# SobeyMIL/MVOC

Hardware: AMD Instinct MI355X
Metric: UNet3D denoising steps/sec, 16x512^2 frames, inversion+compose (higher is better)
Workload: dtype f16

## Files before the change

mvoc_amd/csrc/attention.hip:

```cpp
#include <stdlib.h>

#include "common.h"

namespace {

typedef __fp16 fp16x4_t __attribute__((__vector_size__(4 * sizeof(__fp16))));
template <int D> struct FlashPitch { static constexpr int K = 2 * D + 16, V = D == 64 ? 192 : 320; };

struct AttnArgs {
  const half_t *q, *k, *v;
  half_t* out;
  long q_bs, q_ts, k_bs, k_ts, v_bs, v_ts, o_bs, o_ts;
  int nbatch, heads, tq, tk, kv_bdiv, causal;
  float scale_log2;
  long v2_off, o2_off;
  int qblocks;
};

__device__ __forceinline__ int vt_slot_group(int key) {
  return ((((key >> 5) * 2 + ((key >> 4) & 1)) * 2) + ((key >> 2) & 1));
}
__device__ __forceinline__ int vt_slot_elem(int key) { return ((key >> 3) & 1) * 4 + (key & 3); }

constexpr float FLASH_THR = 8.0f;
// ... 298 lines not shown
      for (int e = 0; e < 16; ++e) ot[v][dt][e] = 0.f;
  float mrun = -INFINITY, lrun = 0.f;
  f32x16 sa[2], sb[2];
  f32x16 zero16;
#pragma unroll
  for (int e = 0; e < 16; ++e) zero16[e] = 0.f;

  int kfo[4];
#pragma unroll
  for (int s = 0; s < 4; ++s) kfo[s] = r * 128 + (((2 * s + h) ^ ((r >> 1) & 7)) * 16);
  const int vq = (lane & 15) >> 2;
  int vfo[2];
#pragma unroll
  for (int dt = 0; dt < 2; ++dt) vfo[dt] = 8192 + (4 * h + vq) * 128 + (((32 * ((lane >> 4) & 1) + 8 * (lane & 3))) | ((dt ^ ((vq >> 1) & 1)) << 6));

  f3_wait_vm<(NS - 2) * PCS>();
  F3_BAR();
#pragma unroll
  for (int t = 0; t < 2; ++t) {
    sa[t] = zero16;
#pragma unroll
    for (int s = 0; s < 4; ++s) {
      const half8_t kf = *reinterpret_cast<const half8_t*>(smem + kfo[s] + 4096 * t);
      sa[t] = __builtin_amdgcn_mfma_f32_32x32x16_f16(kf, qf[s], sa[t], 0, 0, 0);
    }
  }
  int o_v = 0, o_k = TILE, o_w = (NS - 1) * TILE;

  auto body = [&](f32x16(&cur)[2], f32x16(&nxt)[2], const int t) {
    F3_STAMP(4);
    f3_wait_vm<(NS - 3) * PCS>();
    F3_BAR();
    F3_STAMP(0);
    issue(t + NS - 1, o_w);
    F3_FENCE();
    F3_STAMP(1);
    const char* Kn = smem + o_k;
    const char* Vc = smem + o_v;
    if (__builtin_amdgcn_readfirstlane((t == nt - 1) && (p.tk & 63))) {
#pragma unroll
      for (int tt = 0; tt < 2; ++tt)
#pragma unroll
        for (int e = 0; e < 16; ++e)
          if (t * 64 + 32 * tt + 8 * (e >> 2) + 4 * h + (e & 3) >= p.tk) cur[tt][e] = -INFINITY;
    }
    F3_FENCE();
    half8_t kf[2][4];
#pragma unroll
    for (int s = 0; s < 2; ++s)
#pragma unroll
      for (int tt = 0; tt < 2; ++tt) kf[tt][s] = *reinterpret_cast<const half8_t*>(Kn + kfo[s] + 4096 * tt);
    half8_t pf[2];
    half8_t vf[3][NV][2];
    auto vread = [&](const int f) {
#pragma unroll
      for (int v = 0; v < NV; ++v)
#pragma unroll
        for (int dt = 0; dt < 2; ++dt) {
          const char* va = Vc + 8192 * v + vfo[dt] + (32 * (f >> 1) + 16 * (f & 1)) * 128;
          const fp16x4_t lo = __builtin_amdgcn_ds_read_tr16_b64_v4f16((__attribute__((address_space(3))) fp16x4_t*)va);
          const fp16x4_t hi = __builtin_amdgcn_ds_read_tr16_b64_v4f16((__attribute__((address_space(3))) fp16x4_t*)(va + 8 * 128));
#pragma unroll
          for (int e = 0; e < 4; ++e) {
            vf[f % 3][v][dt][e] = (half_t)lo[e];
            vf[f % 3][v][dt][4 + e] = (half_t)hi[e];
          }
        }
    };
    vread(0);
    F3_FENCE();
    auto smma = [&](const int i) {
      const int tt = i & 1, s_ = i >> 1;
      nxt[tt] = __builtin_amdgcn_mfma_f32_32x32x16_f16(kf[tt][s_], qf[s_], s_ == 0 ? zero16 : nxt[tt], 0, 0, 0);
    };
    auto pvmma = [&](const int f, const int dt) {
#pragma unroll
      for (int v = 0; v < NV; ++v) ot[v][dt] = __builtin_amdgcn_mfma_f32_32x32x16_f16(vf[f % 3][v][dt], pf[f & 1], ot[v][dt], 0, 0, 0);
    };
    float mx = fmaxf(cur[0][0], cur[0][1]);
#pragma unroll
    for (int tt = 0; tt < 2; ++tt)
#pragma unroll
      for (int e = tt ? 0 : 2; e < 16; e += 2) mx = __builtin_fmaxf(__builtin_fmaxf(mx, cur[tt][e]), cur[tt][e + 1]);
    smma(0); smma(1); smma(2);
    if constexpr (NV == 2) smma(3);
    mx = flash_xhalf_max(mx);
    if constexpr (NV == 1) { F3_GRP(6, 0); F3_GRP(6, 0); F3_GRP(6, 0); }
    else { F3_GRP(4, 0); F3_GRP(5, 0); F3_GRP(4, 0); F3_GRP(5, 0); }
    F3_STAMP(2);
    if (__any((mx - mrun) * p.scale_log2 > FLASH_THR)) {
      const float mnew = fmaxf(mrun, mx);
      const float alpha = __builtin_amdgcn_exp2f((mrun - mnew) * p.scale_log2);
      mrun = mnew;
      lrun *= alpha;
#pragma unroll
      for (int v = 0; v < NV; ++v)
#pragma unroll
        for (int dt = 0; dt < 2; ++dt)
#pragma unroll
          for (int e = 0; e < 16; ++e) ot[v][dt][e] *= alpha;
    }
    F3_FENCE();
    const f32x2 sc2 = {p.scale_log2, p.scale_log2}, mc2 = {-mrun * p.scale_log2, -mrun * p.scale_log2};
#pragma unroll
    for (int s = 2; s < 4; ++s)
#pragma unroll
      for (int tt = 0; tt < 2; ++tt) kf[tt][s] = *reinterpret_cast<const half8_t*>(Kn + kfo[s] + 4096 * tt);
#pragma unroll
    for (int f = 0; f < 4; ++f) {
      const int tt = f >> 1, s_ = f & 1;
      if (f < 3) vread(f + 1);
      half8_t& pn = pf[f & 1];
      float x[8];
#pragma unroll
      for (int j = 0; j < 8; j += 2) {
        const f32x2 a = __builtin_elementwise_fma(f32x2{cur[tt][8 * s_ + j], cur[tt][8 * s_ + j + 1]}, sc2, mc2);
        x[j] = __builtin_amdgcn_exp2f(a[0]);
        x[j + 1] = __builtin_amdgcn_exp2f(a[1]);
      }
#pragma unroll
      for (int j = 0; j < 8; ++j) pn[j] = (half_t)x[j];
#pragma unroll
      for (int j = 0; j < 4; ++j) lrun = __builtin_amdgcn_fdot2(half2_t{pn[2 * j], pn[2 * j + 1]}, half2_t{(half_t)1.f, (half_t)1.f}, lrun, false);
      if (f == 0) {
        smma(NV == 1 ? 3 : 4); smma(NV == 1 ? 4 : 5);
        if constexpr (NV == 2) { smma(6); smma(7); } else smma(5);
      } else {
        pvmma(f - 1, 0); pvmma(f - 1, 1);
        if constexpr (NV == 1) { if (f < 3) smma(5 + f); }
      }
    }
    pvmma(3, 0);
    pvmma(3, 1);
    if constexpr (NV == 1) {
      F3_RD(8); F3_GRP(5, 3); F3_GRP(5, 2); F3_GRP(5, 3);
      F3_RD(4); F3_GRP(5, 2); F3_GRP(5, 3); F3_GRP(5, 2);
      F3_RD(4); F3_GRP(5, 3); F3_GRP(5, 2); F3_GRP(5, 3);
      F3_GRP(5, 2); F3_GRP(5, 3); F3_GRP(5, 2); F3_GRP(5, 2);
    } else {
      F3_RD(12); F3_GRP(3, 2); F3_GRP(3, 2); F3_GRP(3, 2); F3_GRP(3, 2);
      F3_RD(8); F3_GRP(3, 2); F3_GRP(3, 2); F3_GRP(3, 2); F3_GRP(3, 2);
      F3_RD(8); F3_GRP(3, 2); F3_GRP(3, 2); F3_GRP(3, 2); F3_GRP(3, 2);
      F3_GRP(3, 2); F3_GRP(3, 2); F3_GRP(3, 2); F3_GRP(3, 2);
      F3_GRP(3, 0); F3_GRP(3, 0); F3_GRP(3, 0); F3_GRP(3, 0);
    }
    F3_FENCE();
    F3_STAMP(3);
    const int o_ = o_v; o_v = o_k;
    o_k = o_k + TILE == NS * TILE ? 0 : o_k + TILE;
    o_w = o_;
  };
#pragma unroll 1
  for (int t = 0;; t += 2) {
    body(sa, sb, t);
    if (t + 1 >= nt) break;
    body(sb, sa, t + 1);
    if (t + 2 >= nt) break;
  }
  f3_wait_vm<0>();
#ifdef MVOC_F3_STAMPS
  if (blockIdx.x == 0 && tid == 0) {
    unsigned long long t1_, r1_;
    asm volatile("s_memtime %0\n\ts_memrealtime %1\n\ts_waitcnt lgkmcnt(0)" : "=s"(t1_), "=s"(r1_)::"memory");
    for (int i = 0; i < 5; ++i) f3_dbg[i] = f3_acc[i];
    f3_dbg[5] = t1_ - f3_t0;
    f3_dbg[7] = r1_ - f3_r0;
    f3_dbg[6] = (unsigned long long)nt;
  }
#endif

  const float ltot = lrun + __shfl_xor(lrun, 32);
  const float inv = 1.0f / ltot;
  if (q0 + r < p.tq) {
#pragma unroll
    for (int v = 0; v < NV; ++v) {
      half_t* op = p.out + v * p.o2_off + (long)b * p.o_bs + (long)(q0 + r) * p.o_ts + head * D;
#pragma unroll
      for (int dt = 0; dt < 2; ++dt)
#pragma unroll
        for (int q = 0; q < 4; ++q) {
          half4_t o;
#pragma unroll
          for (int e = 0; e < 4; ++e) o[e] = (half_t)(ot[v][dt][q * 4 + e] * inv);
          *reinterpret_cast<half4_t*>(op + 32 * dt + 8 * q + 4 * h) = o;
        }
    }
  }
}
#undef F3_BAR
#undef F3_FENCE
#undef F3_GRP
#undef F3_RD
#undef F3_STAMP

struct TAttnArgs {
  const half_t *q, *k, *v;
  half_t* out;
  long q_bs, q_ps, q_ts, k_bs, k_ps, k_ts, v_bs, v_ps, v_ts, o_bs, o_ps, o_ts;
  int nsample, hw, heads, frames;
  int logf, logp, pgroups;
  long ntask;
  float scale_log2;
};

constexpr int TVPITCH = 64;

__global__ __launch_bounds__(256) void tattn_kernel(const TAttnArgs p) {
  __shared__ __attribute__((aligned(16))) char smem[4 * 64 * TVPITCH];
  const int tid = threadIdx.x, lane = tid & 63, wave = tid >> 6;
  const int r = lane & 31, h = lane >> 5;
  char* Vs = smem + wave * 64 * TVPITCH;
  const int F = p.frames, logf = p.logf, P = 1 << p.logp;
  const long task = (long)blockIdx.x * 4 + wave;
  const bool active = task < p.ntask;
  const long tk = active ? task : p.ntask - 1;
  const int head = (int)(tk % p.heads);
  const long bp = tk / p.heads;
  const long smp = bp / p.pgroups, px0 = (bp % p.pgroups) << p.logp;
  const half8_t zero8 = {0, 0, 0, 0, 0, 0, 0, 0};
  auto row_px = [&](int row) { return (long)(P > 1 ? row >> logf : 0); };
  auto row_fr = [&](int row) { return P > 1 ? row & (F - 1) : row; };
  auto row_ok = [&](int row) { return (P > 1 || row < F) && px0 + row_px(row) < p.hw; };

  const half_t* qb = p.q + smp * p.q_bs + px0 * p.q_ps + head * 64;
  const half_t* kb = p.k + smp * p.k_bs + px0 * p.k_ps + head * 64;
  const half_t* vb = p.v + smp * p.v_bs + px0 * p.v_ps + head * 64;

#pragma unroll
  for (int i = 0; i < 4; ++i) {
    const int c = lane + 64 * i;
    const int key = c >> 3, dc = c & 7;
    half8_t vr = zero8;
    if (row_ok(key)) vr = *reinterpret_cast<const half8_t*>(vb + row_px(key) * p.v_ps + (long)row_fr(key) * p.v_ts + dc * 8);
    const int g = (((key >> 4) & 1) * 2) + ((key >> 2) & 1), j = vt_slot_elem(key);
#pragma unroll
    for (int e = 0; e < 8; ++e) {
      const int d = dc * 8 + e;
      *reinterpret_cast<half_t*>(Vs + d * TVPITCH + ((g ^ ((d >> 3) & 3)) * 16) + j * 2) = vr[e];
    }
  }
  f32x16 st;
#pragma unroll
  for (int e = 0; e < 16; ++e) st[e] = 0.f;
  const bool rok = row_ok(r);
  const long koff = row_px(r) * p.k_ps + (long)row_fr(r) * p.k_ts, qoff = row_px(r) * p.q_ps + (long)row_fr(r) * p.q_ts;
#pragma unroll
  for (int s = 0; s < 4; ++s) {
    half8_t kf = zero8, qf = zero8;
    if (rok) {
      kf = *reinterpret_cast<const half8_t*>(kb + koff + 16 * s + 8 * h);
      qf = *reinterpret_cast<const half8_t*>(qb + qoff + 16 * s + 8 * h);
    }
    st = __builtin_amdgcn_mfma_f32_32x32x16_f16(kf, qf, st, 0, 0, 0);
  }
  float mx = -INFINITY;
#pragma unroll
  for (int e = 0; e < 16; ++e) {
    const int key = 8 * (e >> 2) + 4 * h + (e & 3);
    const bool ok = P > 1 ? (key >> logf) == (r >> logf) : key < F;
    const float sv = ok ? st[e] * p.scale_log2 : -INFINITY;
    st[e] = sv;
    mx = fmaxf(mx, sv);
  }
  mx = fmaxf(mx, __shfl_xor(mx, 32));
  float ps = 0.f;
#pragma unroll
  for (int e = 0; e < 16; ++e) {
    const float pv = __builtin_amdgcn_exp2f(st[e] - mx);
    st[e] = pv;
    ps += pv;
  }
  ps += __shfl_xor(ps, 32);
  const float inv = 1.0f / ps;

  __syncthreads();
  f32x16 ot[2];
#pragma unroll
  for (int dt = 0; dt < 2; ++dt)
#pragma unroll
    for (int e = 0; e < 16; ++e) ot[dt][e] = 0.f;
#pragma unroll
  for (int s = 0; s < 2; ++s) {
    half8_t pf;
#pragma unroll
    for (int j = 0; j < 8; ++j) pf[j] = (half_t)st[8 * s + j];
    const int g = s * 2 + h;
#pragma unroll
    for (int dt = 0; dt < 2; ++dt) {
      const int d = 32 * dt + r;
      const half8_t vf = *reinterpret_cast<const half8_t*>(Vs + d * TVPITCH + ((g ^ ((d >> 3) & 3)) * 16));
      ot[dt] = __builtin_amdgcn_mfma_f32_32x32x16_f16(vf, pf, ot[dt], 0, 0, 0);
    }
  }
  if (active && rok) {
    half_t* op = p.out + smp * p.o_bs + (px0 + row_px(r)) * p.o_ps + (long)row_fr(r) * p.o_ts + head * 64;
#pragma unroll
    for (int dt = 0; dt < 2; ++dt)
#pragma unroll
      for (int q = 0; q < 4; ++q) {
        half4_t o;
#pragma unroll
        for (int e = 0; e < 4; ++e) o[e] = (half_t)(ot[dt][q * 4 + e] * inv);
        *reinterpret_cast<half4_t*>(op + 32 * dt + 8 * q + 4 * h) = o;
      }
  }
}

}

static const int g_f3_env = getenv("MVOC_FLASH3") ? atoi(getenv("MVOC_FLASH3")) : -1;

extern "C" int mvoc_flash_attn_f16(const mvoc_attn_desc* d, void* stream) {
  MVOC_REQUIRE(d && d->q && d->k && d->v && d->out, -1, "flash_attn: null operand");
  MVOC_REQUIRE(d->nbatch > 0 && d->heads > 0 && d->tq > 0 && d->tk > 0, -1, "flash_attn: empty problem");
  MVOC_REQUIRE(d->nbatch <= 65535 && d->heads <= 65535, -2, "flash_attn: grid too large");
  MVOC_REQUIRE(d->q_ts % 8 == 0 && d->k_ts % 8 == 0 && d->v_ts % 8 == 0 && d->o_ts % 4 == 0, -2,
               "flash_attn: row strides must keep 16-byte alignment");
  AttnArgs a;
  a.q = (const half_t*)d->q; a.k = (const half_t*)d->k; a.v = (const half_t*)d->v; a.out = (half_t*)d->out;
  a.q_bs = d->q_bs; a.q_ts = d->q_ts; a.k_bs = d->k_bs; a.k_ts = d->k_ts; a.v_bs = d->v_bs; a.v_ts = d->v_ts;
  a.o_bs = d->o_bs; a.o_ts = d->o_ts;
  a.nbatch = d->nbatch; a.heads = d->heads; a.tq = d->tq; a.tk = d->tk; a.kv_bdiv = d->kv_bdiv > 0 ? d->kv_bdiv : 1;
  const int hd = d->head_dim > 0 ? d->head_dim : 64;
  MVOC_REQUIRE(hd == 64 || hd == 96, -2, "flash_attn: head_dim (%d) must be 64 or 96", hd);
  MVOC_REQUIRE(!d->causal || d->tq == d->tk, -2, "flash_attn: the causal form is self-attention (tq == tk)");
  a.causal = d->causal;
  a.scale_log2 = (d->scale > 0.f ? d->scale : (hd == 64 ? 0.125f : 1.0f / sqrtf((float)hd))) * 1.4426950408889634f;
  hipStream_t s = (hipStream_t)stream;
  MvocProfScope prof(MVOC_FAM_FLASH, s, (d->v2 ? 2.0 : 1.0) * 4.0 * d->nbatch * d->heads * (double)d->tq * d->tk * hd);
  a.qblocks = (d->tq + 127) / 128;
  const long nblk = (long)a.qblocks * d->heads * d->nbatch;
  MVOC_REQUIRE(nblk < 0x7fffffffL, -2, "flash_attn: grid too large");
  dim3 grid((unsigned)nblk);
  a.v2_off = a.o2_off = 0;
  MVOC_REQUIRE(d->pipelined >= 0 && d->pipelined <= 2, -1, "flash_attn: pipelined must be 0 (by key count), 1 (never) or 2 (wherever it applies)");
  const int f3_mode = d->pipelined ? d->pipelined - 1 : g_f3_env;
  const bool pipelined = hd == 64 && !d->causal && (f3_mode >= 0 ? f3_mode != 0 : d->tk >= 2048);
  if (d->v2) {
    MVOC_REQUIRE(d->out2 && hd == 64, -2, "flash_attn: the paired form needs out2 and head_dim 64");
    a.v2_off = (const half_t*)d->v2 - a.v;
    a.o2_off = (half_t*)d->out2 - a.out;
    MVOC_REQUIRE(a.v2_off % 8 == 0 && a.o2_off % 4 == 0, -2, "flash_attn: v2 / out2 must keep 16-byte alignment");
    if (pipelined) hipLaunchKernelGGL((flash3_kernel<2>), grid, dim3(256), 0, s, a);
    else hipLaunchKernelGGL((flash_kernel<64, 2>), grid, dim3(256), 0, s, a);
  } else if (hd == 64) {
    if (pipelined) hipLaunchKernelGGL((flash3_kernel<1>), grid, dim3(256), 0, s, a);
    else hipLaunchKernelGGL((flash_kernel<64, 1>), grid, dim3(256), 0, s, a);
  } else {
    hipLaunchKernelGGL((flash_kernel<96, 1>), grid, dim3(256), 0, s, a);
  }
  return mvoc_check_launch("flash_kernel");
}

#ifdef MVOC_F3_STAMPS
extern "C" int mvoc_f3_stamps_read(unsigned long long* host8) {
  return hipMemcpyFromSymbol(host8, HIP_SYMBOL(f3_dbg), sizeof(unsigned long long) * 8) == hipSuccess ? 0 : -1;
}
#endif

extern "C" int mvoc_temporal_attn_f16(const mvoc_tattn_desc* d, void* stream) {
  MVOC_REQUIRE(d && d->q && d->k && d->v && d->out, -1, "temporal_attn: null operand");
  MVOC_REQUIRE(d->nsample > 0 && d->hw > 0 && d->heads > 0, -1, "temporal_attn: empty problem");
  MVOC_REQUIRE(d->frames >= 1 && d->frames <= 32, -2, "temporal_attn: frames (%d) must be in [1, 32]", d->frames);
  MVOC_REQUIRE(d->q_ts % 8 == 0 && d->k_ts % 8 == 0 && d->v_ts % 8 == 0 && d->o_ts % 4 == 0 && d->q_ps % 8 == 0 &&
                   d->k_ps % 8 == 0 && d->v_ps % 8 == 0 && d->o_ps % 4 == 0,
               -2, "temporal_attn: strides must keep 16-byte alignment");
  TAttnArgs a;
  a.q = (const half_t*)d->q; a.k = (const half_t*)d->k; a.v = (const half_t*)d->v; a.out = (half_t*)d->out;
  a.q_bs = d->q_bs; a.q_ps = d->q_ps; a.q_ts = d->q_ts; a.k_bs = d->k_bs; a.k_ps = d->k_ps; a.k_ts = d->k_ts;
  a.v_bs = d->v_bs; a.v_ps = d->v_ps; a.v_ts = d->v_ts; a.o_bs = d->o_bs; a.o_ps = d->o_ps; a.o_ts = d->o_ts;
  a.nsample = d->nsample; a.hw = d->hw; a.heads = d->heads; a.frames = d->frames;
  a.logf = d->frames == 8 ? 3 : d->frames == 16 ? 4 : 5;
  a.logp = d->frames == 8 ? 2 : d->frames == 16 ? 1 : 0;
  a.pgroups = (d->hw + (1 << a.logp) - 1) >> a.logp;
  a.ntask = (long)d->nsample * a.pgroups * d->heads;
  a.scale_log2 = 0.125f * 1.4426950408889634f;
  const long nblk = (a.ntask + 3) / 4;
  MVOC_REQUIRE(nblk < 0x7fffffffL, -2, "temporal_attn: grid too large");
  hipStream_t s = (hipStream_t)stream;
  MvocProfScope prof(MVOC_FAM_TATTN, s, 4.0 * (double)d->nsample * d->hw * d->heads * d->frames * 64 * 2);
  hipLaunchKernelGGL(tattn_kernel, dim3((unsigned)nblk), dim3(256), 0, s, a);
  return mvoc_check_launch("tattn_kernel");
}
```

mvoc_amd/csrc/stem.hip:

```cpp
#include "common.h"

namespace {

__global__ void timestep_embedding_kernel(const float* __restrict__ t, int nb, int dim, half_t* __restrict__ out) {
  const int i = blockIdx.x * blockDim.x + threadIdx.x;
  const int half = dim / 2;
  if (i >= nb * dim) return;
  const int b = i / dim, j = i % dim;
  const int k = j < half ? j : j - half;
  const float freq = expf(-logf(10000.0f) * (float)k / (float)half);
  const float ang = t[b] * freq;
  out[i] = (half_t)(j < half ? cosf(ang) : sinf(ang));
}

__global__ void act_kernel(const half_t* __restrict__ x, half_t* __restrict__ out, long n, int act) {
  const long i = (long)blockIdx.x * blockDim.x + threadIdx.x;
  if (i >= n) return;
  const float v = (float)x[i];
  out[i] = (half_t)(act == MVOC_ACT_SILU ? silu_f(v) : act == MVOC_ACT_GELU ? gelu_erf_f(v) : v);
}

__global__ void add_kernel(const half_t* __restrict__ a, const half_t* __restrict__ b, half_t* __restrict__ out, long n) {
  const long i = (long)blockIdx.x * blockDim.x + threadIdx.x;
  if (i >= n) return;
  out[i] = (half_t)((float)a[i] + (float)b[i]);
}

__global__ void conv3x3_small_kernel(const half_t* __restrict__ x, const half_t* __restrict__ w,
                                     const half_t* __restrict__ bias, half_t* __restrict__ out, int nimg, int h, int wd,
                                     int cin, int cout, int stride, int ho, int wo, int silu) {
  const long i = (long)blockIdx.x * blockDim.x + threadIdx.x;
  const long total = (long)nimg * ho * wo * cout;
  if (i >= total) return;
  const int co = (int)(i % cout);
  long pix = i / cout;
  const int ox = (int)(pix % wo);
  pix /= wo;
  const int oy = (int)(pix % ho);
  const int img = (int)(pix / ho);
  float acc = 0.f;
  for (int ky = 0; ky < 3; ++ky) {
    const int iy = oy * stride + ky - 1;
    if (iy < 0 || iy >= h) continue;
    for (int kx = 0; kx < 3; ++kx) {
      const int ix = ox * stride + kx - 1;
      if (ix < 0 || ix >= wd) continue;
      const half_t* xp = x + (((long)img * h + iy) * wd + ix) * cin;
      const half_t* wp = w + ((long)co * 9 + ky * 3 + kx) * cin;
      for (int c = 0; c < cin; ++c) acc += (float)xp[c] * (float)wp[c];
    }
  }
  float v = r16(acc + (bias ? (float)bias[co] : 0.f));
  if (silu) v = silu_f(v);
  out[i] = (half_t)v;
}

__global__ void avgpool_kernel(const half_t* __restrict__ x, half_t* __restrict__ out, int nimg, int h, int w, int c,
                               int oh, int ow) {
  const long i = (long)blockIdx.x * blockDim.x + threadIdx.x;
  const long total = (long)nimg * oh * ow * c;
  if (i >= total) return;
  const int ch = (int)(i % c);
  long pix = i / c;
  const int ox = (int)(pix % ow);
  pix /= ow;
  const int oy = (int)(pix % oh);
  const int img = (int)(pix / oh);
  const int y0 = (oy * h) / oh, y1 = ((oy + 1) * h + oh - 1) / oh;
  const int x0 = (ox * w) / ow, x1 = ((ox + 1) * w + ow - 1) / ow;
  float s = 0.f;
  for (int y = y0; y < y1; ++y)
    for (int xx = x0; xx < x1; ++xx) s += (float)x[(((long)img * h + y) * w + xx) * c + ch];
  out[i] = (half_t)(s / (float)((y1 - y0) * (x1 - x0)));
}

__global__ void ncfhw_to_tokens_kernel(const half_t* __restrict__ x, half_t* __restrict__ out, int b, int c, int f, int hw,
                                       int ldo, int coff) {
  const long i = (long)blockIdx.x * blockDim.x + threadIdx.x;
  const long total = (long)b * f * hw;
  if (i >= total) return;
  const int p = (int)(i % hw);
  const long bf = i / hw;
  const int fi = (int)(bf % f), bi = (int)(bf / f);
  for (int ch = 0; ch < c; ++ch) out[i * ldo + coff + ch] = x[(((long)bi * c + ch) * f + fi) * hw + p];
}

__global__ void tokens_to_ncfhw_kernel(const half_t* __restrict__ x, half_t* __restrict__ out, int b, int c, int f, int hw,
                                       int ld) {
  const long i = (long)blockIdx.x * blockDim.x + threadIdx.x;
  const long total = (long)b * c * f * hw;
  if (i >= total) return;
  const int p = (int)(i % hw);
  long r = i / hw;
  const int fi = (int)(r % f);
  r /= f;
  const int ch = (int)(r % c);
  const int bi = (int)(r / c);
  out[i] = x[(((long)bi * f + fi) * hw + p) * ld + ch];
}

struct Enc4Params {
  half_t ln_g[4], ln_b[4], wq[32], wk[32], wv[32], wo[32], bo[4], w1[64], b1[16], w2[64], b2[4];
};

__device__ __forceinline__ void enc4_ln(const half_t* xp, const Enc4Params& P, float* y) {
  float v[4], mean = 0.f;
#pragma unroll
  for (int c = 0; c < 4; ++c) { v[c] = (float)xp[c]; mean += v[c]; }
  mean *= 0.25f;
  float var = 0.f;
#pragma unroll
  for (int c = 0; c < 4; ++c) var += (v[c] - mean) * (v[c] - mean);
  const float rstd = rsqrtf(var * 0.25f + 1e-5f);
#pragma unroll
  for (int c = 0; c < 4; ++c) y[c] = r16((v[c] - mean) * rstd * (float)P.ln_g[c] + (float)P.ln_b[c]);
}

__global__ void temporal_encoder4_kernel(const half_t* __restrict__ x, const Enc4Params* __restrict__ params,
                                         half_t* __restrict__ out, int b, int f, int hw, int ldo, int coff) {
  __shared__ Enc4Params P;
  for (int i = threadIdx.x; i < (int)(sizeof(Enc4Params) / sizeof(half_t)); i += blockDim.x)
    reinterpret_cast<half_t*>(&P)[i] = reinterpret_cast<const half_t*>(params)[i];
  __syncthreads();
  const long idx = (long)blockIdx.x * blockDim.x + threadIdx.x;
  const long total = (long)b * f * hw;
  if (idx >= total) return;
  const int p = (int)(idx % hw);
  const long bf = idx / hw;
  const int bi = (int)(bf / f);
  const half_t* xi = x + idx * 4;
  float yi[4], q[8];
  enc4_ln(xi, P, yi);
#pragma unroll
  for (int o = 0; o < 8; ++o) {
    float s = 0.f;
#pragma unroll
    for (int c = 0; c < 4; ++c) s += yi[c] * (float)P.wq[o * 4 + c];
    q[o] = r16(s);
  }
  float m[2] = {-INFINITY, -INFINITY}, l[2] = {0.f, 0.f}, acc[8] = {0, 0, 0, 0, 0, 0, 0, 0};
  for (int j = 0; j < f; ++j) {
    const half_t* xj = x + (((long)bi * f + j) * hw + p) * 4;
    float yj[4], k[8], v[8];
    enc4_ln(xj, P, yj);
#pragma unroll
    for (int o = 0; o < 8; ++o) {
      float sk = 0.f, sv = 0.f;
#pragma unroll
      for (int c = 0; c < 4; ++c) {
        sk += yj[c] * (float)P.wk[o * 4 + c];
        sv += yj[c] * (float)P.wv[o * 4 + c];
      }
      k[o] = r16(sk);
      v[o] = r16(sv);
    }
#pragma unroll
    for (int hd = 0; hd < 2; ++hd) {
      float s = 0.f;
#pragma unroll
      for (int d = 0; d < 4; ++d) s += q[hd * 4 + d] * k[hd * 4 + d];
      s *= 0.5f;
      const float mn = fmaxf(m[hd], s);
      const float a = __expf(m[hd] - mn), pj = __expf(s - mn);
      l[hd] = l[hd] * a + pj;
#pragma unroll
      for (int d = 0; d < 4; ++d) acc[hd * 4 + d] = acc[hd * 4 + d] * a + pj * v[hd * 4 + d];
      m[hd] = mn;
    }
  }
  float att[8];
#pragma unroll
  for (int o = 0; o < 8; ++o) att[o] = r16(acc[o] / l[o >> 2]);
  float h1[4];
#pragma unroll
  for (int c = 0; c < 4; ++c) {
    float s = 0.f;
#pragma unroll
    for (int o = 0; o < 8; ++o) s += att[o] * (float)P.wo[c * 8 + o];
    h1[c] = r16(r16(s + (float)P.bo[c]) + (float)xi[c]);
  }
  float ff[16];
#pragma unroll
  for (int o = 0; o < 16; ++o) {
    float s = 0.f;
#pragma unroll
    for (int c = 0; c < 4; ++c) s += h1[c] * (float)P.w1[o * 4 + c];
    ff[o] = r16(gelu_erf_f(r16(s + (float)P.b1[o])));
  }
#pragma unroll
  for (int c = 0; c < 4; ++c) {
    float s = 0.f;
#pragma unroll
    for (int o = 0; o < 16; ++o) s += ff[o] * (float)P.w2[c * 16 + o];
    out[idx * ldo + coff + c] = (half_t)(r16(s + (float)P.b2[c]) + h1[c]);
  }
}

__global__ void delay_kernel(long ticks) {
  const long t0 = __builtin_amdgcn_s_memrealtime();
  while ((long)__builtin_amdgcn_s_memrealtime() - t0 < ticks) __builtin_amdgcn_s_sleep(32);
}

inline unsigned nblk(long n, int bs = 256) { return (unsigned)((n + bs - 1) / bs); }

__global__ __launch_bounds__(256) void clip_patches_kernel(const half_t* __restrict__ x, half_t* __restrict__ out, int size, int patch,
                                                           int kpad, long total) {
  const long i = (long)blockIdx.x * 256 + threadIdx.x;
  if (i >= total) return;
  const int g = size / patch;
  const int k = (int)(i % kpad);
  const long row = i / kpad;
  half_t v = (half_t)0.f;
  if (k < 3 * patch * patch) {
    const int c = k / (patch * patch), py = (k / patch) % patch, px = k % patch;
    const int gx = (int)(row % g), gy = (int)((row / g) % g);
    const long b = row / ((long)g * g);
    v = x[((b * 3 + c) * size + gy * patch + py) * (long)size + gx * patch + px];
  }
  out[i] = v;
}

__global__ __launch_bounds__(256) void clip_embed_kernel(const half_t* __restrict__ table, const int* __restrict__ ids,
                                                         const half_t* __restrict__ cls, const half_t* __restrict__ pos,
                                                         half_t* __restrict__ out, int T, int c8n, long total) {
  const long i = (long)blockIdx.x * 256 + threadIdx.x;
  if (i >= total) return;
  const int c8 = (int)(i % c8n);
  const long row = i / c8n;
  const int t = (int)(row % T);
  const half_t* src;
  if (ids) src = table + ((long)ids[row] * c8n + c8) * 8;
  else if (t == 0) src = cls + c8 * 8;
  else src = table + (((row / T) * (T - 1) + t - 1) * c8n + c8) * 8;
  const half8_t a = *reinterpret_cast<const half8_t*>(src);
  const half8_t b = *reinterpret_cast<const half8_t*>(pos + ((long)t * c8n + c8) * 8);
  half8_t o;
#pragma unroll
  for (int e = 0; e < 8; ++e) o[e] = (half_t)((float)a[e] + (float)b[e]);
  reinterpret_cast<half8_t*>(out)[i] = o;
}

}

extern "C" int mvoc_timestep_embedding_f16(const float* t_dev, int32_t nb, int32_t dim, void* out, void* stream) {
  MVOC_REQUIRE(t_dev && out && nb > 0 && dim > 0 && dim % 2 == 0, -1, "timestep_embedding: bad args");
  hipStream_t s = (hipStream_t)stream;
  MvocProfScope prof(MVOC_FAM_MISC, s, 2.0 * nb * dim);
  hipLaunchKernelGGL(timestep_embedding_kernel, dim3(nblk((long)nb * dim)), dim3(256), 0, s, t_dev, nb, dim, (half_t*)out);
  return mvoc_check_launch("timestep_embedding_kernel");
}

extern "C" int mvoc_act_f16(const void* x, void* out, int64_t n, int32_t act, void* stream) {
  MVOC_REQUIRE(x && out && n > 0, -1, "act: bad args");
  hipStream_t s = (hipStream_t)stream;
  MvocProfScope prof(MVOC_FAM_MISC, s, 4.0 * n);
  hipLaunchKernelGGL(act_kernel, dim3(nblk(n)), dim3(256), 0, s, (const half_t*)x, (half_t*)out, (long)n, act);
  return mvoc_check_launch("act_kernel");
}

extern "C" int mvoc_add_f16(const void* a, const void* b, void* out, int64_t n, void* stream) {
  MVOC_REQUIRE(a && b && out && n > 0, -1, "add: bad args");
  hipStream_t s = (hipStream_t)stream;
  MvocProfScope prof(MVOC_FAM_MISC, s, 6.0 * n);
  hipLaunchKernelGGL(add_kernel, dim3(nblk(n)), dim3(256), 0, s, (const half_t*)a, (const half_t*)b, (half_t*)out, (long)n);
  return mvoc_check_launch("add_kernel");
}

extern "C" int mvoc_conv3x3_small_f16(const void* x, const void* w, const void* bias, void* out, int32_t nimg, int32_t h,
                                      int32_t wd, int32_t cin, int32_t cout, int32_t stride, int32_t silu, void* stream) {
  MVOC_REQUIRE(x && w && out && nimg > 0 && h > 0 && wd > 0 && cin > 0 && cout > 0 && (stride == 1 || stride == 2), -1,
               "conv3x3_small: bad args");
  const int ho = (h + 2 - 3) / stride + 1, wo = (wd + 2 - 3) / stride + 1;
  const long total = (long)nimg * ho * wo * cout;
  hipStream_t s = (hipStream_t)stream;
  MvocProfScope prof(MVOC_FAM_MISC, s, 2.0 * ((double)nimg * h * wd * cin + total));
  hipLaunchKernelGGL(conv3x3_small_kernel, dim3(nblk(total)), dim3(256), 0, s, (const half_t*)x, (const half_t*)w,
                     (const half_t*)bias, (half_t*)out, nimg, h, wd, cin, cout, stride, ho, wo, silu);
  return mvoc_check_launch("conv3x3_small_kernel");
}

__global__ void conv1x1_small_kernel(const half_t* __restrict__ x, const half_t* __restrict__ w, const half_t* __restrict__ bias,
                                     half_t* __restrict__ out, long rows, int cin, int cout) {
  const long i = (long)blockIdx.x * blockDim.x + threadIdx.x;
  if (i >= rows * cout) return;
  const int co = (int)(i % cout);
  const long r = i / cout;
  float acc = 0.f;
  for (int c = 0; c < cin; ++c) acc += (float)x[r * cin + c] * (float)w[co * cin + c];
  out[i] = (half_t)(acc + (bias ? (float)bias[co] : 0.f));
}

__global__ void image_to_tokens_kernel(const half_t* __restrict__ x, half_t* __restrict__ out, int n, int c, int hw) {
  const long i = (long)blockIdx.x * blockDim.x + threadIdx.x;
  if (i >= (long)n * hw * c) return;
  const int ch = (int)(i % c);
  const long px = i / c;
  const int img = (int)(px / hw), p = (int)(px % hw);
  out[i] = x[((long)img * c + ch) * hw + p];
}
__global__ void tokens_to_image_kernel(const half_t* __restrict__ x, half_t* __restrict__ out, int n, int c, int hw, int ld) {
  const long i = (long)blockIdx.x * blockDim.x + threadIdx.x;
  if (i >= (long)n * c * hw) return;
  const int p = (int)(i % hw);
  const long t = i / hw;
  const int ch = (int)(t % c), img = (int)(t / c);
  out[i] = x[((long)img * hw + p) * ld + ch];
}

__global__ void gaussian_sample_kernel(const half_t* __restrict__ mean, const half_t* __restrict__ logvar,
                                       const half_t* __restrict__ noise, half_t* __restrict__ out, long n) {
  const long i = (long)blockIdx.x * blockDim.x + threadIdx.x;
  if (i >= n) return;
  const float lv = fminf(fmaxf((float)logvar[i], -30.0f), 20.0f);
  const float sd = r16(expf(r16(0.5f * lv)));
  out[i] = (half_t)((float)mean[i] + r16(sd * (float)noise[i]));
}
__global__ void scale_kernel(const half_t* __restrict__ x, half_t* __restrict__ out, long n, float s) {
  const long i = (long)blockIdx.x * blockDim.x + threadIdx.x;
  if (i >= n) return;
  float p = s * (float)x[i];
  asm volatile("" : "+v"(p));
  out[i] = (half_t)p;
}

extern "C" int mvoc_gaussian_sample_f16(const void* mean, const void* logvar, const void* noise, void* out, int64_t n, void* stream) {
  MVOC_REQUIRE(mean && logvar && noise && out && n > 0, -1, "gaussian_sample: bad args");
  hipStream_t s = (hipStream_t)stream;
  MvocProfScope prof(MVOC_FAM_MISC, s, 8.0 * n);
  hipLaunchKernelGGL(gaussian_sample_kernel, dim3(nblk(n)), dim3(256), 0, s, (const half_t*)mean, (const half_t*)logvar,
                     (const half_t*)noise, (half_t*)out, (long)n);
  return mvoc_check_launch("gaussian_sample_kernel");
}

extern "C" int mvoc_clip_patches_f16(const void* pixels, void* out, int32_t nimg, int32_t size, int32_t patch, int32_t kpad,
                                     void* stream) {
  MVOC_REQUIRE(pixels && out && nimg > 0 && patch > 0 && size > 0 && size % patch == 0 && kpad >= 3 * patch * patch, -1,
               "clip_patches: bad args");
  const long total = (long)nimg * (size / patch) * (size / patch) * kpad;
  hipStream_t s = (hipStream_t)stream;
  MvocProfScope prof(MVOC_FAM_MISC, s, 4.0 * total);
  hipLaunchKernelGGL(clip_patches_kernel, dim3(nblk(total)), dim3(256), 0, s, (const half_t*)pixels, (half_t*)out, size, patch, kpad, total);
  return mvoc_check_launch("clip_patches_kernel");
}

extern "C" int mvoc_clip_embed_f16(const void* table, const int32_t* ids, const void* cls, const void* pos, void* out, int64_t rows,
                                   int32_t t, int32_t c, void* stream) {
  MVOC_REQUIRE(table && pos && out && rows > 0 && t > 0 && rows % t == 0 && c > 0 && c % 8 == 0 && (ids || cls), -1,
               "clip_embed: bad args (c %% 8, rows %% t, ids or cls)");
  const long total = rows * (c / 8);
  hipStream_t s = (hipStream_t)stream;
  MvocProfScope prof(MVOC_FAM_MISC, s, 6.0 * rows * c);
  hipLaunchKernelGGL(clip_embed_kernel, dim3(nblk(total)), dim3(256), 0, s, (const half_t*)table, (const int*)ids, (const half_t*)cls,
                     (const half_t*)pos, (half_t*)out, t, c / 8, total);
  return mvoc_check_launch("clip_embed_kernel");
}

extern "C" int mvoc_scale_f16(const void* x, void* out, int64_t n, double scale, void* stream) {
  MVOC_REQUIRE(x && out && n > 0, -1, "scale: bad args");
  hipStream_t s = (hipStream_t)stream;
  MvocProfScope prof(MVOC_FAM_MISC, s, 4.0 * n);
  hipLaunchKernelGGL(scale_kernel, dim3(nblk(n)), dim3(256), 0, s, (const half_t*)x, (half_t*)out, (long)n, (float)scale);
  return mvoc_check_launch("scale_kernel");
}

extern "C" int mvoc_conv1x1_small_f16(const void* x, const void* w, const void* bias, void* out, int64_t rows, int32_t cin,
                                      int32_t cout, void* stream) {
  MVOC_REQUIRE(x && w && out && rows > 0 && cin > 0 && cout > 0 && cin <= 64 && cout <= 64, -1, "conv1x1_small: bad args");
  hipStream_t s = (hipStream_t)stream;
  MvocProfScope prof(MVOC_FAM_MISC, s, 2.0 * rows * (cin + cout));
  hipLaunchKernelGGL(conv1x1_small_kernel, dim3(nblk(rows * cout)), dim3(256), 0, s, (const half_t*)x, (const half_t*)w,
                     (const half_t*)bias, (half_t*)out, (long)rows, cin, cout);
  return mvoc_check_launch("conv1x1_small_kernel");
}

extern "C" int mvoc_image_to_tokens_f16(const void* x, void* out, int32_t n, int32_t c, int32_t hw, void* stream) {
  MVOC_REQUIRE(x && out && n > 0 && c > 0 && hw > 0, -1, "image_to_tokens: bad args");
  hipStream_t s = (hipStream_t)stream;
  MvocProfScope prof(MVOC_FAM_MISC, s, 4.0 * n * c * hw);
  hipLaunchKernelGGL(image_to_tokens_kernel, dim3(nblk((long)n * c * hw)), dim3(256), 0, s, (const half_t*)x, (half_t*)out, n, c, hw);
  return mvoc_check_launch("image_to_tokens_kernel");
}

extern "C" int mvoc_tokens_to_image_f16(const void* x, void* out, int32_t n, int32_t c, int32_t hw, int32_t ld, void* stream) {
  MVOC_REQUIRE(x && out && n > 0 && c > 0 && hw > 0 && ld >= c, -1, "tokens_to_image: bad args");
  hipStream_t s = (hipStream_t)stream;
  MvocProfScope prof(MVOC_FAM_MISC, s, 4.0 * n * c * hw);
  hipLaunchKernelGGL(tokens_to_image_kernel, dim3(nblk((long)n * c * hw)), dim3(256), 0, s, (const half_t*)x, (half_t*)out, n, c, hw, ld);
  return mvoc_check_launch("tokens_to_image_kernel");
}

__global__ void resize8_pass_kernel(const uint8_t* __restrict__ in, uint8_t* __restrict__ out, const int* __restrict__ bounds,
                                    const int* __restrict__ kk, int ksize, long nimg, int olen, int other, long in_img, long out_img,
                                    long in_si, long in_so, long out_si, long out_so) {
  const long i = (long)blockIdx.x * blockDim.x + threadIdx.x;
  if (i >= nimg * olen * other) return;
  const int xx = (int)(i % olen);
  const long t = i / olen;
  const int o = (int)(t % other);
  const long img = t / other;
  const int xmin = bounds[2 * xx], n = bounds[2 * xx + 1];
  const uint8_t* src = in + img * in_img + (long)o * in_so + (long)xmin * in_si;
  int acc = 1 << 21;
  for (int x = 0; x < n; ++x) acc += (int)src[(long)x * in_si] * kk[xx * ksize + x];
  acc >>= 22;
  out[img * out_img + (long)o * out_so + (long)xx * out_si] = (uint8_t)(acc < 0 ? 0 : acc > 255 ? 255 : acc);
}
__global__ void mask_finish_kernel(const uint8_t* __restrict__ v, half_t* __restrict__ fl, uint8_t* __restrict__ bl, long n) {
  const long i = (long)blockIdx.x * blockDim.x + threadIdx.x;
  if (i >= n) return;
  const int x = v[i];
  fl[i] = (half_t)((float)x / 255.0f);
  bl[i] = x > 10 ? 1 : 0;
}

extern "C" int mvoc_mask_resize_u8(const void* in, void* tmp, void* out, int32_t n, int32_t H, int32_t W, int32_t h, int32_t w,
                                   const int32_t* bounds_h, const int32_t* kk_h, int32_t ksize_h, const int32_t* bounds_v,
                                   const int32_t* kk_v, int32_t ksize_v, void* stream) {
  MVOC_REQUIRE(in && tmp && out && bounds_h && kk_h && bounds_v && kk_v && n > 0 && H > 0 && W > 0 && h > 0 && w > 0, -1, "mask_resize: bad args");
  hipStream_t s = (hipStream_t)stream;
  MvocProfScope prof(MVOC_FAM_MISC, s, (double)n * H * W + 2.0 * n * H * w + (double)n * h * w);
  hipLaunchKernelGGL(resize8_pass_kernel, dim3(nblk((long)n * H * w)), dim3(256), 0, s, (const uint8_t*)in, (uint8_t*)tmp, bounds_h, kk_h,
                     ksize_h, (long)n, w, H, (long)H * W, (long)H * w, 1L, (long)W, 1L, (long)w);
  hipLaunchKernelGGL(resize8_pass_kernel, dim3(nblk((long)n * h * w)), dim3(256), 0, s, (const uint8_t*)tmp, (uint8_t*)out, bounds_v, kk_v,
                     ksize_v, (long)n, h, w, (long)H * w, (long)h * w, (long)w, 1L, (long)w, 1L);
  return mvoc_check_launch("resize8_pass_kernel");
}

extern "C" int mvoc_mask_finish(const void* v, void* float_mask, void* bool_mask, int64_t n, void* stream) {
  MVOC_REQUIRE(v && float_mask && bool_mask && n > 0, -1, "mask_finish: bad args");
  hipStream_t s = (hipStream_t)stream;
  MvocProfScope prof(MVOC_FAM_MISC, s, 4.0 * n);
  hipLaunchKernelGGL(mask_finish_kernel, dim3(nblk(n)), dim3(256), 0, s, (const uint8_t*)v, (half_t*)float_mask, (uint8_t*)bool_mask, (long)n);
  return mvoc_check_launch("mask_finish_kernel");
}

__global__ void permute_rows_kernel(const half_t* __restrict__ x, half_t* __restrict__ out, int d1, int d2, int d3, long s0, long s1,
                                    long s2, long s3, int c8n, long total) {
  const long i = (long)blockIdx.x * blockDim.x + threadIdx.x;
  if (i >= total) return;
  const int c8 = (int)(i % c8n);
  long r = i / c8n;
  const int i3 = (int)(r % d3); r /= d3;
  const int i2 = (int)(r % d2); r /= d2;
  const int i1 = (int)(r % d1);
  const long i0 = r / d1;
  const long src = i0 * s0 + i1 * s1 + i2 * s2 + i3 * s3;
  reinterpret_cast<half8_t*>(out)[i] = *reinterpret_cast<const half8_t*>(x + (src * c8n + c8) * 8);
}

extern "C" int mvoc_permute_rows_f16(const void* x, void* out, const int64_t* dims4, const int64_t* strides4, int32_t c, void* stream) {
  MVOC_REQUIRE(x && out && dims4 && strides4 && c > 0 && c % 8 == 0, -1, "permute_rows: bad args (c %% 8)");
  for (int k = 0; k < 4; ++k) MVOC_REQUIRE(dims4[k] > 0 && dims4[k] < (1 << 30), -1, "permute_rows: bad dim");
  const long total = (long)dims4[0] * dims4[1] * dims4[2] * dims4[3] * (c / 8);
  hipStream_t s = (hipStream_t)stream;
  MvocProfScope prof(MVOC_FAM_MISC, s, 32.0 * total);
  hipLaunchKernelGGL(permute_rows_kernel, dim3(nblk(total)), dim3(256), 0, s, (const half_t*)x, (half_t*)out, (int)dims4[1], (int)dims4[2],
                     (int)dims4[3], (long)strides4[0], (long)strides4[1], (long)strides4[2], (long)strides4[3], c / 8, total);
  return mvoc_check_launch("permute_rows_kernel");
}

extern "C" int mvoc_adaptive_avgpool_f16(const void* x, void* out, int32_t nimg, int32_t h, int32_t w, int32_t c,
                                         int32_t oh, int32_t ow, void* stream) {
  MVOC_REQUIRE(x && out && nimg > 0 && h > 0 && w > 0 && c > 0 && oh > 0 && ow > 0, -1, "avgpool: bad args");
  const long total = (long)nimg * oh * ow * c;
  hipStream_t s = (hipStream_t)stream;
  MvocProfScope prof(MVOC_FAM_MISC, s, 2.0 * ((double)nimg * h * w * c + total));
  hipLaunchKernelGGL(avgpool_kernel, dim3(nblk(total)), dim3(256), 0, s, (const half_t*)x, (half_t*)out, nimg, h, w, c, oh,
                     ow);
  return mvoc_check_launch("avgpool_kernel");
}

extern "C" int mvoc_ncfhw_to_tokens_f16(const void* x, void* out, int32_t b, int32_t c, int32_t f, int32_t hw, int32_t ldo,
                                        int32_t coff, void* stream) {
  MVOC_REQUIRE(x && out && b > 0 && c > 0 && f > 0 && hw > 0 && ldo >= coff + c, -1, "ncfhw_to_tokens: bad args");
  hipStream_t s = (hipStream_t)stream;
  MvocProfScope prof(MVOC_FAM_MISC, s, 4.0 * b * c * f * hw);
  hipLaunchKernelGGL(ncfhw_to_tokens_kernel, dim3(nblk((long)b * f * hw)), dim3(256), 0, s, (const half_t*)x,
                     (half_t*)out, b, c, f, hw, ldo, coff);
  return mvoc_check_launch("ncfhw_to_tokens_kernel");
}

extern "C" int mvoc_tokens_to_ncfhw_f16(const void* x, void* out, int32_t b, int32_t c, int32_t f, int32_t hw, int32_t ld,
                                        void* stream) {
  MVOC_REQUIRE(x && out && b > 0 && c > 0 && f > 0 && hw > 0 && ld >= c, -1, "tokens_to_ncfhw: bad args");
  hipStream_t s = (hipStream_t)stream;
  MvocProfScope prof(MVOC_FAM_MISC, s, 4.0 * b * c * f * hw);
  hipLaunchKernelGGL(tokens_to_ncfhw_kernel, dim3(nblk((long)b * c * f * hw)), dim3(256), 0, s, (const half_t*)x,
                     (half_t*)out, b, c, f, hw, ld);
  return mvoc_check_launch("tokens_to_ncfhw_kernel");
}

extern "C" int mvoc_temporal_encoder4_f16(const void* x, const void* params, void* out, int32_t b, int32_t f, int32_t hw,
                                          int32_t ldo, int32_t coff, void* stream) {
  MVOC_REQUIRE(x && params && out && b > 0 && f > 0 && hw > 0 && ldo >= coff + 4, -1, "temporal_encoder4: bad args");
  hipStream_t s = (hipStream_t)stream;
  MvocProfScope prof(MVOC_FAM_MISC, s, 16.0 * b * f * hw);
  hipLaunchKernelGGL(temporal_encoder4_kernel, dim3(nblk((long)b * f * hw)), dim3(256), 0, s, (const half_t*)x,
                     (const Enc4Params*)params, (half_t*)out, b, f, hw, ldo, coff);
  return mvoc_check_launch("temporal_encoder4_kernel");
}

extern "C" int mvoc_delay_us(int64_t us, void* stream) {
  MVOC_REQUIRE(us >= 0 && us <= 2000000, -1, "delay_us: out of range");
  hipLaunchKernelGGL(delay_kernel, dim3(1), dim3(64), 0, (hipStream_t)stream, (long)us * 100);
  return mvoc_check_launch("delay_kernel");
}
```

Measured before the change: 21.57.

## Add single-pass MFMA temporal attention kernel and vectorize elementwise add

Adds a temporal-attention kernel in which each wave handles up to 32 frame rows. It computes QK^T with one chain of 32x32x16 MFMAs, applies a block-diagonal mask per pixel, and does the softmax in registers using a permlane32 swap for the cross-half sum. V is staged in LDS and read back with transposing ds_read_tr16 loads for the PV MFMA. The new path is on by default whenever more than one pixel is packed per task and the strides fit in 32-bit offsets, which removes the older kernel's per-element overhead. Separately, the elementwise add gains a 16-byte vectorized grid-stride kernel with a scalar tail launch, which may cost an extra launch for odd sizes.

```diff
diff --git a/mvoc_amd/csrc/attention.hip b/mvoc_amd/csrc/attention.hip
--- a/mvoc_amd/csrc/attention.hip
+++ b/mvoc_amd/csrc/attention.hip
@@ -624,6 +624,120 @@
 #pragma unroll
         for (int e = 0; e < 4; ++e) o[e] = (half_t)(ot[dt][q * 4 + e] * inv);
         *reinterpret_cast<half4_t*>(op + 32 * dt + 8 * q + 4 * h) = o;
+      }
+  }
+}
+
+constexpr int TSPITCH = 192;
+
+__device__ __forceinline__ float tattn_xhalf_sum(float x) {
+  const unsigned u = __builtin_bit_cast(unsigned, x);
+  const auto sw = __builtin_amdgcn_permlane32_swap(u, u, false, false);
+  return __builtin_bit_cast(float, (unsigned)sw[0]) + __builtin_bit_cast(float, (unsigned)sw[1]);
+}
+
+__global__ __launch_bounds__(256) void stream_tattn_kernel(const TAttnArgs p) {
+  __shared__ __attribute__((aligned(16))) char smem[4 * 32 * TSPITCH];
+  const int tid = threadIdx.x, lane = tid & 63;
+  const int wave = __builtin_amdgcn_readfirstlane(tid >> 6);
+  const int r = lane & 31, h = lane >> 5;
+  char* Vs = smem + wave * 32 * TSPITCH;
+  const int F = p.frames, logf = p.logf, logp = p.logp;
+  const unsigned task = blockIdx.x * 4u + (unsigned)wave;
+  if (task >= (unsigned)p.ntask) return;
+
+  const unsigned head = task % (unsigned)p.heads, bp = task / (unsigned)p.heads;
+  const unsigned smp = bp / (unsigned)p.pgroups, px0 = (bp % (unsigned)p.pgroups) << logp;
+  const char* qb = reinterpret_cast<const char*>(p.q + (long)smp * p.q_bs + (long)px0 * p.q_ps + head * 64);
+  const char* kb = reinterpret_cast<const char*>(p.k + (long)smp * p.k_bs + (long)px0 * p.k_ps + head * 64);
+  const char* vb = reinterpret_cast<const char*>(p.v + (long)smp * p.v_bs + (long)px0 * p.v_ps + head * 64);
+  char* ob = reinterpret_cast<char*>(p.out + (long)smp * p.o_bs + (long)px0 * p.o_ps + head * 64);
+  const int npx = min(1 << logp, p.hw - (int)px0);
+
+  const int rpx = r >> logf, rfr = r & (F - 1), rpx_c = rpx < npx ? rpx : 0;
+  const unsigned qoff = ((unsigned)rpx_c * (unsigned)p.q_ps + (unsigned)rfr * (unsigned)p.q_ts) * 2u + 16u * h;
+  const unsigned koff = ((unsigned)rpx_c * (unsigned)p.k_ps + (unsigned)rfr * (unsigned)p.k_ts) * 2u + 16u * h;
+  const unsigned ooff = ((unsigned)rpx * (unsigned)p.o_ps + (unsigned)rfr * (unsigned)p.o_ts) * 2u + 8u * h;
+  const half8_t zero8 = {0, 0, 0, 0, 0, 0, 0, 0};
+  half8_t kf[4], qf[4], vr[4];
+#pragma unroll
+  for (int i = 0; i < 4; ++i) {
+    const int key = (lane >> 3) + 8 * i, kpx = key >> logf, kpx_c = kpx < npx ? kpx : 0;
+    const unsigned voff = ((unsigned)kpx_c * (unsigned)p.v_ps + (unsigned)(key & (F - 1)) * (unsigned)p.v_ts) * 2u + 16u * (lane & 7);
+    vr[i] = *reinterpret_cast<const half8_t*>(vb + voff);
+  }
+#pragma unroll
+  for (int s = 0; s < 4; ++s) {
+    kf[s] = *reinterpret_cast<const half8_t*>(kb + koff + 32 * s);
+    qf[s] = *reinterpret_cast<const half8_t*>(qb + qoff + 32 * s);
+  }
+#pragma unroll
+  for (int i = 0; i < 4; ++i)
+    if ((((lane >> 3) + 8 * i) >> logf) >= npx) vr[i] = zero8;
+  char* vst = Vs + (lane >> 3) * TSPITCH + (lane & 7) * 16;
+#pragma unroll
+  for (int i = 0; i < 4; ++i) *reinterpret_cast<half8_t*>(vst + 8 * i * TSPITCH) = vr[i];
+  f32x16 st;
+#pragma unroll
+  for (int e = 0; e < 16; ++e) st[e] = 0.f;
+#pragma unroll
+  for (int s = 0; s < 4; ++s) st = __builtin_amdgcn_mfma_f32_32x32x16_f16(kf[s], qf[s], st, 0, 0, 0);
+  float mx = -INFINITY;
+#pragma unroll
+  for (int e = 0; e < 16; ++e) {
+    const int key = 8 * (e >> 2) + 4 * h + (e & 3);
+    const bool ok = (key >> logf) == (r >> logf);
+    const float sv = ok ? st[e] * p.scale_log2 : -INFINITY;
+    st[e] = sv;
+    mx = fmaxf(mx, sv);
+  }
+  mx = flash_xhalf_max(mx);
+  float ps = 0.f;
+#pragma unroll
+  for (int e = 0; e < 16; ++e) {
+    const float pv = __builtin_amdgcn_exp2f(st[e] - mx);
+    st[e] = pv;
+    ps += pv;
+  }
+  ps = tattn_xhalf_sum(ps);
+  const float inv = 1.0f / ps;
+
+  asm volatile("" ::: "memory");
+  f32x16 ot[2];
+#pragma unroll
+  for (int dt = 0; dt < 2; ++dt)
+#pragma unroll
+    for (int e = 0; e < 16; ++e) ot[dt][e] = 0.f;
+  const char* vld = Vs + (4 * h + ((lane & 15) >> 2)) * TSPITCH + (16 * ((lane >> 4) & 1) + 4 * (lane & 3)) * 2;
+#pragma unroll
+  for (int s = 0; s < 2; ++s) {
+    half8_t pf;
+#pragma unroll
+    for (int j = 0; j < 8; ++j) pf[j] = (half_t)st[8 * s + j];
+#pragma unroll
+    for (int dt = 0; dt < 2; ++dt) {
+      const char* va = vld + 16 * s * TSPITCH + 64 * dt;
+      const fp16x4_t lo = __builtin_amdgcn_ds_read_tr16_b64_v4f16((__attribute__((address_space(3))) fp16x4_t*)va);
+      const fp16x4_t hi = __builtin_amdgcn_ds_read_tr16_b64_v4f16((__attribute__((address_space(3))) fp16x4_t*)(va + 8 * TSPITCH));
+      half8_t vf;
+#pragma unroll
+      for (int e = 0; e < 4; ++e) {
+        vf[e] = (half_t)lo[e];
+        vf[4 + e] = (half_t)hi[e];
+      }
+      ot[dt] = __builtin_amdgcn_mfma_f32_32x32x16_f16(vf, pf, ot[dt], 0, 0, 0);
+    }
+  }
+  if (rpx < npx) {
+    half_t* op = reinterpret_cast<half_t*>(ob + ooff);
+#pragma unroll
+    for (int dt = 0; dt < 2; ++dt)
+#pragma unroll
+      for (int q = 0; q < 4; ++q) {
+        half4_t o;
+#pragma unroll
+        for (int e = 0; e < 4; ++e) o[e] = (half_t)(ot[dt][q * 4 + e] * inv);
+        *reinterpret_cast<half4_t*>(op + 32 * dt + 8 * q) = o;
       }
   }
 }
@@ -680,6 +794,8 @@
 }
 #endif
 
+static const int g_tattn_stream = getenv("MVOC_TATTN_STREAM") ? atoi(getenv("MVOC_TATTN_STREAM")) : 1;
+
 extern "C" int mvoc_temporal_attn_f16(const mvoc_tattn_desc* d, void* stream) {
   MVOC_REQUIRE(d && d->q && d->k && d->v && d->out, -1, "temporal_attn: null operand");
   MVOC_REQUIRE(d->nsample > 0 && d->hw > 0 && d->heads > 0, -1, "temporal_attn: empty problem");
@@ -701,6 +817,13 @@
   MVOC_REQUIRE(nblk < 0x7fffffffL, -2, "temporal_attn: grid too large");
   hipStream_t s = (hipStream_t)stream;
   MvocProfScope prof(MVOC_FAM_TATTN, s, 4.0 * (double)d->nsample * d->hw * d->heads * d->frames * 64 * 2);
+  const int P = 1 << a.logp;
+  auto span = [&](long ps, long ts) { return ps >= 0 && ts >= 0 && ((P - 1) * ps + (d->frames - 1) * ts + 64) * 2 < 0x7fffffffL; };
+  if (g_tattn_stream && a.logp > 0 && a.ntask < 0x7fffffffL && span(d->q_ps, d->q_ts) && span(d->k_ps, d->k_ts) &&
+      span(d->v_ps, d->v_ts) && span(d->o_ps, d->o_ts)) {
+    hipLaunchKernelGGL(stream_tattn_kernel, dim3((unsigned)nblk), dim3(256), 0, s, a);
+    return mvoc_check_launch("stream_tattn_kernel");
+  }
   hipLaunchKernelGGL(tattn_kernel, dim3((unsigned)nblk), dim3(256), 0, s, a);
   return mvoc_check_launch("tattn_kernel");
 }
diff --git a/mvoc_amd/csrc/stem.hip b/mvoc_amd/csrc/stem.hip
--- a/mvoc_amd/csrc/stem.hip
+++ b/mvoc_amd/csrc/stem.hip
@@ -24,6 +24,18 @@
   const long i = (long)blockIdx.x * blockDim.x + threadIdx.x;
   if (i >= n) return;
   out[i] = (half_t)((float)a[i] + (float)b[i]);
+}
+
+__global__ __launch_bounds__(256) void add8_kernel(const half8_t* __restrict__ a, const half8_t* __restrict__ b,
+                                                   half8_t* __restrict__ out, long n8) {
+  const long step = (long)gridDim.x * 256;
+  for (long i = (long)blockIdx.x * 256 + threadIdx.x; i < n8; i += step) {
+    const half8_t x = a[i], y = b[i];
+    half8_t o;
+#pragma unroll
+    for (int e = 0; e < 8; ++e) o[e] = (half_t)((float)x[e] + (float)y[e]);
+    out[i] = o;
+  }
 }
 
 __global__ void conv3x3_small_kernel(const half_t* __restrict__ x, const half_t* __restrict__ w,
@@ -262,7 +274,16 @@
   MVOC_REQUIRE(a && b && out && n > 0, -1, "add: bad args");
   hipStream_t s = (hipStream_t)stream;
   MvocProfScope prof(MVOC_FAM_MISC, s, 6.0 * n);
-  hipLaunchKernelGGL(add_kernel, dim3(nblk(n)), dim3(256), 0, s, (const half_t*)a, (const half_t*)b, (half_t*)out, (long)n);
+  const half_t *pa = (const half_t*)a, *pb = (const half_t*)b;
+  half_t* po = (half_t*)out;
+  const long n8 = (((uintptr_t)a | (uintptr_t)b | (uintptr_t)out) & 15) == 0 ? (long)(n / 8) : 0;
+  if (n8 > 0) {
+    const long blocks = (n8 + 255) / 256;
+    hipLaunchKernelGGL(add8_kernel, dim3((unsigned)(blocks < 8192 ? blocks : 8192)), dim3(256), 0, s, (const half8_t*)pa,
+                       (const half8_t*)pb, (half8_t*)po, n8);
+  }
+  const long done = n8 * 8, rest = (long)n - done;
+  if (rest > 0) hipLaunchKernelGGL(add_kernel, dim3(nblk(rest)), dim3(256), 0, s, pa + done, pb + done, po + done, rest);
   return mvoc_check_launch("add_kernel");
 }
 
```

Measured after the change: 21.60, median of 4. No clear change (+0.1%).
